# lmb-freiburg/neural-point-cloud-diffusion

Measured on AMD Instinct MI355X. Metric: denoiser train steps/sec (+ rendered rays/sec under 'render'), SRN-Cars 512pt x 128d, higher is better.
Workload: dtype bf16; 1 GPU; BASELINE configs[1]: denoiser fwd/bwd + AdamW + EMA, 512 points x 128-d latents, width 1024 / 24 layers / 16 heads (seq 513), bf16 autocast; global_batch=64, per_gpu_batch=64, parallelism=dp1, rng=weights seed 1234 on every rank; timestep / noise draws seed 42 + rank

## Files before the change

### include/npcd_hip.h

```cpp
#ifndef NPCD_HIP_H
#define NPCD_HIP_H

#include <stdint.h>

#ifdef __cplusplus
extern "C" {
#endif

#define NPCD_OK 0
#define NPCD_ERR_ARG (-1)
#define NPCD_ERR_UNSUPPORTED (-2)
#define NPCD_ERR_HIP (-3)

#define NPCD_BF16 0
#define NPCD_F16 1
#define NPCD_F32 2

int npcd_abi_version(void);
const char* npcd_error_string(int code);
const char* npcd_last_hip_error(void);

int npcd_attn_fwd(const void* q, const void* k, const void* v, void* out, float* lse,
                  int B, int n, int H, int d,
                  int64_t qkv_sb, int64_t qkv_sn, int64_t qkv_sh,
// ... 146 lines not shown
typedef struct NpcdColsumJob {
    const float* part;
    float* out;
    int nblk, N, accumulate, reserved;
} NpcdColsumJob;
int npcd_colsum_finalize_batch(const NpcdColsumJob* jobs, int njobs, void* stream);
int npcd_gelu_fwd(const void* h, void* g, int64_t numel, void* stream);
int npcd_colsum_blocks(int T);
int npcd_gelu_bwd(const void* dg, const void* h, void* dh, float* part, int T, int N, void* stream);
int npcd_colsum_bf16(const void* a, float* part, int T, int N, void* stream);
int npcd_small_wgrad_blocks(int T);
int npcd_small_wgrad(const void* dy, const void* x, float* part, int T, int J, int K, void* stream);
int npcd_adamw_ema(float* p, float* g, float* m, float* v, float* ema, void* shadow_bf16, int64_t numel,
                   float lr, float beta1, float beta2, float eps, float weight_decay, int step,
                   float ema_decay, int zero_grad, void* stream);
int npcd_cast_f32_bf16(const float* src, void* dst, int64_t numel, void* stream);
int npcd_add_ln_fwd_dt(const float* x_in, const void* delta, const float* gamma, const float* beta,
                       float* x_out, void* y, float* mean, float* rstd, int T, int W, float eps, int dtype, void* stream);
int npcd_ln_bwd_dt(const void* dy, const float* x, const float* mean, const float* rstd, const float* gamma,
                   const float* dres, float* dx, void* dxb, float* part_gamma, float* part_beta,
                   float* part_col, int T, int W, int dtype, void* stream);
int npcd_gelu_fwd_dt(const void* h, void* g, int64_t numel, int dtype, void* stream);
int npcd_gelu_bwd_dt(const void* dg, const void* h, void* dh, float* part, int T, int N, int dtype, void* stream);
int npcd_colsum_dt(const void* a, float* part, int T, int N, int dtype, void* stream);
int npcd_adamw_ema_dt(float* p, float* g, float* m, float* v, float* ema, void* shadow, int shadow_dtype, int64_t numel,
                      float lr, float beta1, float beta2, float eps, float weight_decay, int step,
                      float ema_decay, int zero_grad, void* stream);
int npcd_cast_f32_dt(const float* src, void* dst, int64_t numel, int dtype, void* stream);

typedef struct NpcdScalerCtl {
    int32_t found_inf, step, growth_tracker, skipped;
    float loss_scale, inv_scale, grad_norm, clip_coef, bc1, bc2_sqrt;
    int32_t reserved[6];
} NpcdScalerCtl;
int npcd_grad_stats_blocks(void);
int npcd_grad_stats(const float* g, int64_t n, double* work, double* out, void* stream);
int npcd_scaler_finalize(const double* stats, int nslots, NpcdScalerCtl* ctl, int scaling, int clip, float max_norm,
                         float beta1, float beta2, float growth_factor, float backoff_factor, int growth_interval, void* stream);
int npcd_adamw_ema_gated(float* p, float* g, float* m, float* v, float* ema, void* shadow, int shadow_dtype, int64_t numel,
                         float lr, float beta1, float beta2, float eps, float weight_decay, double ema_decay, int zero_grad,
                         const NpcdScalerCtl* ctl, void* stream);

int npcd_wgrad_slices(int T, int N, int K);
int npcd_wgrad(const void* dy, const void* x, float* out, float* workspace, int T, int N, int K, int dtype, void* stream);
int npcd_wgrad_group(int count, const void* const* dy, const void* const* x, float* const* out, const int* N, const int* K, int T,
                     int dtype, void* stream);

int npcd_linear_fwd(const void* x, const void* w, const void* bias, void* y, int M, int N, int K, int dtype, void* stream);
int npcd_linear_gelu_fwd(const void* x, const void* w, const void* bias, void* h, void* g, int M, int N, int K, int dtype, void* stream);
int npcd_linear_dgelu_rows(int M);
int npcd_linear_dgelu_bwd(const void* dy, const void* wt, const void* h, void* dh, float* part, int M, int N, int K, int dtype, void* stream);
int npcd_linear128_fwd(const void* x, const void* w, const void* bias, void* y, int M, int N, int K, int dtype, void* stream);
int npcd_transpose_16(const void* in, void* out, int R, int C, void* stream);

int npcd_sum_slices(const float* part, float* out, int S, int64_t numel, void* stream);

int npcd_ddpm_reverse_step(const float* x_t, const void* eps, int eps_dtype, const float* noise, float* x_prev, float* x0_out,
                           const int64_t* t, int B, int64_t per_sample, const float* tab_recip, const float* tab_recipm1,
                           const float* tab_coef1, const float* tab_coef2, const float* tab_logvar, float clip_lo, float clip_hi,
                           int has_clip, void* stream);

int npcd_q_sample(const float* x0, const float* noise, const int64_t* t, const float* tab_sqrt_acp, const float* tab_sqrt_1macp,
                  float* x_t, int B, int64_t per_sample, void* stream);
int npcd_eps_mse_blocks(void);
int npcd_eps_mse_fwd(const float* noise, const void* eps, int eps_dtype, int64_t numel, float* pointwise, float* part, float* loss,
                     void* stream);
int npcd_eps_mse_bwd(const float* noise, const void* eps, int eps_dtype, int64_t numel, const float* upstream_dev, void* grad,
                     void* stream);

int npcd_ray_march_compact(const float* sigma, const float* rgb, const uint64_t* ray_bits, const float* pts,
                           const int32_t* ray_base, const float* rays_o, const float* rays_d, const float* t1,
                           int Nr, int M, int capacity, int white_back, float* mask, float* depth, float* channels,
                           float* depth_ws, void* stream);

int64_t npcd_render_lim_words(int B, int R);
int npcd_render_rays_query(const npcd_grid_params* grid, const void* workspace, const float* points, int B, int N, const float* extr,
                           const float* intr, int views, int res, float box, int S, int M, int k, float r, float* rays_o, float* rays_d,
                           float* t0, float* t1, int32_t* counter, int32_t capacity, int32_t* ray_base, int32_t* ray_nsel,
                           uint64_t* ray_bits, int32_t* nb_idx, float* pts, void* order_ws, uint32_t* lim_part, void* stream);
int npcd_ray_march_compact_fused(const float* sigma, const float* rgb, const uint64_t* ray_bits, const float* pts, const int32_t* ray_base,
                                 const float* rays_o, const float* rays_d, const float* t0, const float* t1, const uint32_t* lim_part,
                                 int lim_pairs, int Nr, int M, int capacity, int white_back, float* mask, float* depth,
                                 float* channels, float* depth_ws, void* stream);

int npcd_pair_input_fwd(const int64_t* flat, const int64_t* owner, const float* pts, const float* kp_pos, const float* kp_feat,
                        int feat_dim, int n_freqs, int64_t n_pairs, float* x0, float* w, void* stream);
int npcd_pair_input_bwd(const int64_t* flat, const float* dx0, int feat_dim, int n_cols, int64_t n_pairs, float* dfeat, void* stream);
int npcd_leaky_bwd_blocks(int64_t rows);
int npcd_leaky_bwd_colsum(const void* dz, const void* z, void* dy, float* part, int64_t rows, int N, float slope, int dtype,
                          void* stream);
int npcd_pair_aggregate(int backward, const float* src, const float* w, const int64_t* off, const int64_t* cnt, int channels,
                        int64_t n_points, float* dst, void* stream);

#define NPCD_PAIR_MLP_BF16 0
#define NPCD_PAIR_MLP_X2 1
int64_t npcd_pair_mlp_wpack_bytes(int feat_dim, int precision);
int npcd_pair_mlp_pack(const float* const* weights_dev, const float* const* biases_dev, int feat_dim, int precision, void* wpack_dev,
                       void* stream);
int npcd_pair_mlp_fwd(const void* wpack, int feat_dim, int precision, const int64_t* nb_idx, const float* pts, const float* kp_pos,
                      const float* kp_feat, const int64_t* off, int64_t n_points, int k, int64_t n_pairs, void* x0, void* acts,
                      float* wn, float* G, void* stream);
int npcd_pair_mlp_bwd_slabs(int64_t n_pairs, int precision);
int64_t npcd_pair_mlp_bwd_workspace_floats(int feat_dim, int64_t n_pairs, int precision);
int npcd_pair_mlp_bwd(const void* wpack, int feat_dim, int precision, const float* dG, const int64_t* owner, const float* wn,
                      const void* x0, const void* acts, int64_t n_pairs, void* dact, float* dfeat, float* part, float* const* dW,
                      float* const* db, void* stream);
// ... 26 lines not shown
```

### neural-point-cloud-diffusion_amd/csrc/gemm_nt.hip

```cpp
#include <type_traits>

#include "common.h"

namespace npcd {

__device__ __forceinline__ uint32_t l_lds_addr(const unsigned char* p) {
    return (uint32_t)(uintptr_t)(__attribute__((address_space(3))) const unsigned char*)p;
}
__device__ __forceinline__ const void* l_uniform_ptr(const void* p) {
    const uint64_t v = reinterpret_cast<uint64_t>(p);
    const uint32_t lo = __builtin_amdgcn_readfirstlane((uint32_t)v), hi = __builtin_amdgcn_readfirstlane((uint32_t)(v >> 32));
    return reinterpret_cast<const void*>(((uint64_t)hi << 32) | lo);
}
__device__ __forceinline__ void l_dma16(const void* sbase, uint32_t voff, uint32_t lds_dst) {
    sbase = l_uniform_ptr(sbase);
    asm volatile("s_mov_b32 m0, %2\n\ts_nop 0\n\tglobal_load_lds_dwordx4 %0, %1" ::"v"(voff), "s"(sbase), "s"(lds_dst) : "memory");
}
__device__ __forceinline__ void l_dma16_lane(const void* src, uint32_t lds_dst) {
    asm volatile("s_mov_b32 m0, %1\n\ts_nop 0\n\tglobal_load_lds_dwordx4 %0, off" ::"v"(src), "s"(lds_dst) : "memory");
}
template <int OFF>
__device__ __forceinline__ u32x4 l_rd128(uint32_t addr) {
    u32x4 v;
    asm volatile("ds_read_b128 %0, %1 offset:%2" : "=v"(v) : "v"(addr), "n"(OFF) : "memory");
// ... 539 lines not shown
#pragma unroll
    for (int ni = 0; ni < 2; ++ni) {
        const int nb = n0 + 64 * wn + 32 * ni;
        float bq[4][4];
#pragma unroll
        for (int q = 0; q < 4; ++q) {
            if (bias) lin_unpack4<TR>(*reinterpret_cast<const u32x2*>(bias + nb + 8 * q + 4 * h), bq[q]);
            else bq[q][0] = bq[q][1] = bq[q][2] = bq[q][3] = 0.f;
        }
#pragma unroll
        for (int mi = 0; mi < MB; ++mi) {
            if (mi >= mb_store) continue;
            const int m = m0 + xrow0 + 32 * mi + r;
            const bool ok = m < p.M;
            const int64_t rowoff = (int64_t)(ok ? m : 0) * p.N + nb + 8 * h;
#pragma unroll
            for (int qp = 0; qp < 2; ++qp) {
                float v[2][4];
#pragma unroll
                for (int e = 0; e < 2; ++e)
#pragma unroll
                    for (int j = 0; j < 4; ++j) v[e][j] = acc[ni][mi][4 * (2 * qp + e) + j] + bq[2 * qp + e][j];
                const uint32_t a0 = lin_pack2<E>(v[0][0], v[0][1]), a1 = lin_pack2<E>(v[0][2], v[0][3]);
                const uint32_t b0 = lin_pack2<E>(v[1][0], v[1][1]), b1 = lin_pack2<E>(v[1][2], v[1][3]);
                const auto s0 = __builtin_amdgcn_permlane32_swap(a0, b0, false, false);
                const auto s1 = __builtin_amdgcn_permlane32_swap(a1, b1, false, false);
                if (ok) *reinterpret_cast<u32x4*>(Y + rowoff + 16 * qp) = u32x4{s0[0], s1[0], s0[1], s1[1]};
            }
        }
    }
}

template <class TR>
__global__ __launch_bounds__(512, 2) void lin128_kernel(Lin128Params p) {
    extern __shared__ __attribute__((aligned(16))) unsigned char smem[];
    const int l = xcd_remap(blockIdx.x, gridDim.x);
    const int tn = l % p.tiles_n, tm = l / p.tiles_n;
    if (p.tall && tm == p.tiles_m - 1) lin128_tile<TR, 3>(p, smem, tm, tn);
    else lin128_tile<TR, 2>(p, smem, tm, tn);
}

template <class E>
__global__ __launch_bounds__(256) void transpose16_kernel(const E* __restrict__ in, E* __restrict__ out, int R, int C) {
    __shared__ E tile[64][66];
    const int c0 = blockIdx.x * 64, r0 = blockIdx.y * 64;
    const int tx = threadIdx.x & 63, ty = threadIdx.x >> 6;
    for (int i = ty; i < 64; i += 4)
        if (r0 + i < R && c0 + tx < C) tile[i][tx] = in[(int64_t)(r0 + i) * C + c0 + tx];
    __syncthreads();
    for (int i = ty; i < 64; i += 4)
        if (c0 + i < C && r0 + tx < R) out[(int64_t)(c0 + i) * R + r0 + tx] = tile[tx][i];
}

}

using namespace npcd;

static int lin_cus() {
    static const int n = [] {
        int dev = 0, cu = 256;
        if (hipGetDevice(&dev) == hipSuccess && hipDeviceGetAttribute(&cu, hipDeviceAttributeMultiprocessorCount, dev) != hipSuccess) cu = 256;
        const char* e = getenv("NPCD_LIN_GRID");
        return e ? atoi(e) : cu;
    }();
    return n;
}

template <class TR, int EPI>
static int lin_launch(const LinParams& p, hipStream_t st) {
    static DynLds lds;
    const void* k = reinterpret_cast<const void*>(lin_kernel<TR, EPI>);
    NPCD_HIP_CHECK(lds.ensure(k, kLRing));
    const int grid = p.ntiles < lin_cus() ? p.ntiles : lin_cus();
    hipLaunchKernelGGL((lin_kernel<TR, EPI>), dim3(grid), dim3(512), kLRing, st, p);
    NPCD_HIP_CHECK(hipGetLastError());
    return NPCD_OK;
}

static int lin_common(int epi, const void* x, const void* w, const void* bias, void* y, void* y2, const void* aux, float* part, int M, int N, int K,
                      int dtype, void* stream) {
    if (!x || !w || !y || M <= 0 || N <= 0 || K <= 0) return NPCD_ERR_ARG;
    if (N % 256 || (N / 256) % 4 || K % 64 || (dtype != NPCD_BF16 && dtype != NPCD_F16)) return NPCD_ERR_UNSUPPORTED;
    if ((int64_t)M * N >= (int64_t)1 << 31 || (int64_t)M * K >= (int64_t)1 << 31) return NPCD_ERR_UNSUPPORTED;
    for (const void* q : {x, w, bias, (const void*)y, (const void*)y2, aux})
        if (reinterpret_cast<uintptr_t>(q) & 15) return NPCD_ERR_ARG;
    if (epi == LIN_GELU && !y2) return NPCD_ERR_ARG;
    if (epi == LIN_DGELU && (!aux || !part || bias)) return NPCD_ERR_ARG;
    LinParams p{};
    p.x = x; p.w = w; p.bias = bias; p.y = y; p.y2 = y2; p.aux = aux; p.part = part;
    p.M = M; p.N = N; p.K = K;
    p.tiles_m = (M + 255) / 256; p.tiles_n = N / 256;
    p.ntiles = p.tiles_m * p.tiles_n;
    p.full_m = p.tiles_m / 8 * 8;
    hipStream_t st = static_cast<hipStream_t>(stream);
#define NPCD_LIN_GO(TRT)                                                          \
    switch (epi) {                                                                \
        case LIN_PLAIN: return lin_launch<TRT, LIN_PLAIN>(p, st);                 \
        case LIN_GELU: return lin_launch<TRT, LIN_GELU>(p, st);                   \
        default: return lin_launch<TRT, LIN_DGELU>(p, st);                        \
    }
    if (dtype == NPCD_BF16) { NPCD_LIN_GO(BF16) }
    NPCD_LIN_GO(F16)
#undef NPCD_LIN_GO
}

extern "C" int npcd_linear_fwd(const void* x, const void* w, const void* bias, void* y, int M, int N, int K, int dtype, void* stream) {
    return lin_common(LIN_PLAIN, x, w, bias, y, nullptr, nullptr, nullptr, M, N, K, dtype, stream);
}
extern "C" int npcd_linear_gelu_fwd(const void* x, const void* w, const void* bias, void* h, void* g, int M, int N, int K, int dtype, void* stream) {
    return lin_common(LIN_GELU, x, w, bias, h, g, nullptr, nullptr, M, N, K, dtype, stream);
}
extern "C" int npcd_linear_dgelu_rows(int M) { return M <= 0 ? -1 : 2 * ((M + 255) / 256); }
extern "C" int npcd_linear_dgelu_bwd(const void* dy, const void* wt, const void* h, void* dh, float* part, int M, int N, int K, int dtype,
                                     void* stream) {
    return lin_common(LIN_DGELU, dy, wt, nullptr, dh, nullptr, h, part, M, N, K, dtype, stream);
}
extern "C" int npcd_linear128_fwd(const void* x, const void* w, const void* bias, void* y, int M, int N, int K, int dtype, void* stream) {
    if (!x || !w || !y || M <= 0 || N <= 0 || K <= 0) return NPCD_ERR_ARG;
    if (N % 128 || K % 64 || (dtype != NPCD_BF16 && dtype != NPCD_F16)) return NPCD_ERR_UNSUPPORTED;
    if ((int64_t)M * N >= (int64_t)1 << 31 || (int64_t)M * K >= (int64_t)1 << 30 || (int64_t)N * K >= (int64_t)1 << 30) return NPCD_ERR_UNSUPPORTED;
    for (const void* q : {x, w, bias, (const void*)y})
        if (reinterpret_cast<uintptr_t>(q) & 15) return NPCD_ERR_ARG;
    Lin128Params p{};
    p.x = x; p.w = w; p.bias = bias; p.y = y;
    p.M = M; p.N = N; p.K = K;
    const int rem = M % 128;
    p.tall = (M > 128 && rem >= 1 && rem <= 32) ? 128 + rem : 0;
    p.tiles_m = p.tall ? M / 128 : (M + 127) / 128;
    p.tiles_n = N / 128;
    hipStream_t st = static_cast<hipStream_t>(stream);
    static DynLds lds_b, lds_h;
    const int grid = p.tiles_m * p.tiles_n;
    if (dtype == NPCD_BF16) {
        NPCD_HIP_CHECK(lds_b.ensure(reinterpret_cast<const void*>(lin128_kernel<BF16>), kL128Lds));
        hipLaunchKernelGGL(lin128_kernel<BF16>, dim3(grid), dim3(512), kL128Lds, st, p);
    } else {
        NPCD_HIP_CHECK(lds_h.ensure(reinterpret_cast<const void*>(lin128_kernel<F16>), kL128Lds));
        hipLaunchKernelGGL(lin128_kernel<F16>, dim3(grid), dim3(512), kL128Lds, st, p);
    }
    NPCD_HIP_CHECK(hipGetLastError());
    return NPCD_OK;
}
#ifdef NPCD_L128_TL
extern "C" int npcd_lin128_debug_read(long long* out, int count) {
    return (int)hipMemcpyFromSymbol(out, HIP_SYMBOL(npcd::g_l128_tl), sizeof(long long) * count);
}
#endif
#ifdef NPCD_LIN_TL
extern "C" int npcd_lin_debug_read(long long* out, int count) {
    return (int)hipMemcpyFromSymbol(out, HIP_SYMBOL(npcd::g_lin_tl), sizeof(long long) * count);
}
#endif
extern "C" int npcd_transpose_16(const void* in, void* out, int R, int C, void* stream) {
    if (!in || !out || R <= 0 || C <= 0) return NPCD_ERR_ARG;
    hipLaunchKernelGGL(transpose16_kernel<uint16_t>, dim3((C + 63) / 64, (R + 63) / 64), dim3(256), 0, static_cast<hipStream_t>(stream),
                       static_cast<const uint16_t*>(in), static_cast<uint16_t*>(out), R, C);
    NPCD_HIP_CHECK(hipGetLastError());
    return NPCD_OK;
}
```

### neural-point-cloud-diffusion_amd/npcd/hip/__init__.py

```python
import ctypes
import os
from ctypes import POINTER, c_char_p, c_double, c_float, c_int, c_int32, c_int64, c_void_p

import torch

_PKG_ROOT = os.path.dirname(os.path.dirname(os.path.dirname(os.path.abspath(__file__))))
LIB_PATH = os.environ.get("NPCD_HIP_LIB") or os.path.join(_PKG_ROOT, "lib", "libnpcd_hip.so")

NPCD_BF16, NPCD_F16, NPCD_F32 = 0, 1, 2
NPCD_GRID_FINE, NPCD_GRID_SCALED = 0, 1
_DTYPE_CODE = {torch.bfloat16: NPCD_BF16, torch.float16: NPCD_F16, torch.float32: NPCD_F32}


class GridParams(ctypes.Structure):
    _fields_ = [("voxel_size", c_float * 3), ("voxel_scale", c_int32 * 3), ("kernel_size", c_int32 * 3),
                ("max_points_per_voxel", c_int32), ("max_occ_voxels_per_example", c_int32),
                ("range_min", c_float * 3), ("range_max", c_float * 3), ("dims", c_int32 * 3), ("cdims", c_int32 * 3),
                ("grid_level", c_int32)]


_P = c_void_p
SIGNATURES = {
    "npcd_abi_version": (c_int, []),
    "npcd_error_string": (c_char_p, [c_int]),
# ... 30 lines not shown
    "npcd_ray_march_compact_fused": (c_int, [_P] * 10 + [c_int, c_int, c_int, c_int, c_int] + [_P] * 4 + [_P]),
    "npcd_ray_gen": (c_int, [_P, _P, c_int, c_int, c_float] + [_P] * 5 + [_P]),
    "npcd_ray_gen_subset": (c_int, [_P, _P, c_int, c_int, c_float, _P, c_int] + [_P] * 5 + [_P]),
    "npcd_shade_wpack_bytes": (c_int64, [c_int, c_int, c_int]),
    "npcd_shade_workspace_bytes": (c_int64, [c_int, c_int]),
    "npcd_shade_pack_weights": (c_int, [POINTER(_P), POINTER(_P), c_int, c_int, c_int, _P]),
    "npcd_pairs_x2_wpack_bytes": (c_int64, [c_int]),
    "npcd_pairs_x2_pack": (c_int, [POINTER(_P), POINTER(_P), c_int, _P]),
    "npcd_pairs_x2": (c_int, [_P, c_int, _P, _P, _P, _P, _P, c_int, c_int, _P, _P]),
    "npcd_points_x2_wpack_bytes": (c_int64, []),
    "npcd_points_x2_pack": (c_int, [POINTER(_P), POINTER(_P), c_int, _P]),
    "npcd_points_x2": (c_int, [_P, _P, _P, c_int, _P, _P, _P, _P, _P]),
    "npcd_points_x2_train": (c_int, [_P, _P, c_int, _P, _P, _P]),
    "npcd_points_x2_pack_dev": (c_int, [POINTER(_P), POINTER(_P), c_int, _P, _P]),
    "npcd_shade_points": (c_int, [_P, c_int, c_int, c_int] + [_P] * 5 + [c_int, c_int] + [_P] * 3 + [_P] + [_P]),
    "npcd_shade_points_dir": (c_int, [_P, c_int, c_int, c_int] + [_P] * 5 + [c_int, c_int] + [_P] * 3 + [_P, _P] + [_P] + [_P]),
    "npcd_ray_march_ws_floats": (c_int64, [c_int]),
    "npcd_ray_gen_ws_floats": (c_int64, [c_int, c_int, c_int]),
    "npcd_ray_march": (c_int, [_P] * 8 + [c_int, c_int, c_int] + [_P] * 4 + [_P]),
    "npcd_add_ln_fwd": (c_int, [_P] * 8 + [c_int, c_int, c_float, _P]),
    "npcd_ln_bwd_blocks": (c_int, [c_int]),
    "npcd_ln_bwd": (c_int, [_P] * 11 + [c_int, c_int, _P]),
    "npcd_colsum_scratch_rows": (c_int, []),
    "npcd_colsum_finalize": (c_int, [_P, c_int, c_int, _P, c_int, _P]),
    "npcd_colsum_finalize_batch": (c_int, [_P, c_int, _P]),
    "npcd_ddpm_reverse_step": (c_int, [_P, _P, c_int, _P, _P, _P, _P, c_int, c_int64, _P, _P, _P, _P, _P, c_float, c_float, c_int, _P]),
    "npcd_gelu_fwd": (c_int, [_P, _P, c_int64, _P]),
    "npcd_colsum_blocks": (c_int, [c_int]),
    "npcd_gelu_bwd": (c_int, [_P, _P, _P, _P, c_int, c_int, _P]),
    "npcd_colsum_bf16": (c_int, [_P, _P, c_int, c_int, _P]),
    "npcd_adamw_ema": (c_int, [_P] * 6 + [c_int64] + [c_float] * 5 + [c_int, c_float, c_int, _P]),
    "npcd_cast_f32_bf16": (c_int, [_P, _P, c_int64, _P]),
    "npcd_add_ln_fwd_dt": (c_int, [_P] * 8 + [c_int, c_int, c_float, c_int, _P]),
    "npcd_ln_bwd_dt": (c_int, [_P] * 11 + [c_int, c_int, c_int, _P]),
    "npcd_gelu_fwd_dt": (c_int, [_P, _P, c_int64, c_int, _P]),
    "npcd_gelu_bwd_dt": (c_int, [_P, _P, _P, _P, c_int, c_int, c_int, _P]),
    "npcd_colsum_dt": (c_int, [_P, _P, c_int, c_int, c_int, _P]),
    "npcd_adamw_ema_dt": (c_int, [_P] * 6 + [c_int, c_int64] + [c_float] * 5 + [c_int, c_float, c_int, _P]),
    "npcd_cast_f32_dt": (c_int, [_P, _P, c_int64, c_int, _P]),
    "npcd_grad_stats_blocks": (c_int, []),
    "npcd_grad_stats": (c_int, [_P, c_int64, _P, _P, _P]),
    "npcd_scaler_finalize": (c_int, [_P, c_int, _P, c_int, c_int] + [c_float] * 5 + [c_int, _P]),
    "npcd_adamw_ema_gated": (c_int, [_P] * 6 + [c_int, c_int64] + [c_float] * 5 + [c_double, c_int, _P, _P]),
    "npcd_wgrad_slices": (c_int, [c_int, c_int, c_int]),
    "npcd_wgrad": (c_int, [_P, _P, _P, _P, c_int, c_int, c_int, c_int, _P]),
    "npcd_wgrad_group": (c_int, [c_int, POINTER(_P), POINTER(_P), POINTER(_P), POINTER(c_int), POINTER(c_int), c_int, c_int, _P]),
    "npcd_sum_slices": (c_int, [_P, _P, c_int, c_int64, _P]),
    "npcd_linear_fwd": (c_int, [_P, _P, _P, _P, c_int, c_int, c_int, c_int, _P]),
    "npcd_linear128_fwd": (c_int, [_P, _P, _P, _P, c_int, c_int, c_int, c_int, _P]),
    "npcd_linear_gelu_fwd": (c_int, [_P, _P, _P, _P, _P, c_int, c_int, c_int, c_int, _P]),
    "npcd_linear_dgelu_rows": (c_int, [c_int]),
    "npcd_linear_dgelu_bwd": (c_int, [_P, _P, _P, _P, _P, c_int, c_int, c_int, c_int, _P]),
    "npcd_transpose_16": (c_int, [_P, _P, c_int, c_int, _P]),
    "npcd_small_wgrad_blocks": (c_int, [c_int]),
    "npcd_small_wgrad": (c_int, [_P, _P, _P, c_int, c_int, c_int, _P]),
    "npcd_q_sample": (c_int, [_P] * 6 + [c_int, c_int64, _P]),
    "npcd_eps_mse_blocks": (c_int, []),
    "npcd_eps_mse_fwd": (c_int, [_P, _P, c_int, c_int64, _P, _P, _P, _P]),
    "npcd_eps_mse_bwd": (c_int, [_P, _P, c_int, c_int64, _P, _P, _P]),
    "npcd_split3_bf16": (c_int, [_P, _P, _P, c_int64, c_int, c_int, _P]),
    "npcd_add_ln_split3_bf16": (c_int, [_P] * 7 + [c_int64, c_int, c_float, _P]),
    "npcd_add_ln_split3_stats_bf16": (c_int, [_P] * 9 + [c_int64, c_int, c_float, _P]),
    "npcd_split_weights_bf16": (c_int, [_P, c_int, _P]),
    "npcd_ln_bwd_split3_bf16": (c_int, [_P] * 11 + [c_int, c_int, _P]),
    "npcd_split3_colsum_bf16": (c_int, [_P] * 5 + [c_int, c_int, c_int, _P]),
    "npcd_pair_mlp_wpack_bytes": (c_int64, [c_int, c_int]),
    "npcd_pair_mlp_pack": (c_int, [POINTER(_P), POINTER(_P), c_int, c_int, _P, _P]),
    "npcd_pair_mlp_fwd": (c_int, [_P, c_int, c_int] + [_P] * 5 + [c_int64, c_int, c_int64] + [_P] * 4 + [_P]),
    "npcd_pair_mlp_bwd_slabs": (c_int, [c_int64, c_int]),
    "npcd_pair_mlp_bwd_workspace_floats": (c_int64, [c_int, c_int64, c_int]),
    "npcd_pair_mlp_bwd": (c_int, [_P, c_int, c_int] + [_P] * 5 + [c_int64] + [_P] * 3 + [POINTER(_P), POINTER(_P), _P]),
}

_lib = None


def lib() -> ctypes.CDLL:
    global _lib
    if _lib is None:
        if not os.path.exists(LIB_PATH):
            raise RuntimeError(
                f"libnpcd_hip.so not found at {LIB_PATH}: build it with "
                f"`python neural-point-cloud-diffusion_amd/csrc/build.py` (or __graft_entry__.build()). "
                f"There is no CPU / PyTorch fallback for the NPCD hot path.")
        handle = ctypes.CDLL(LIB_PATH)
        missing = []
        for name, (res, args) in SIGNATURES.items():
            try:
                fn = getattr(handle, name)
            except AttributeError:
                missing.append(name)
                continue
            fn.restype, fn.argtypes = res, args
        handle.npcd_missing = tuple(missing)
        _lib = handle
    return _lib


def check(rc: int, what: str):
    if rc != 0:
        L = lib()
        msg = L.npcd_error_string(rc).decode()
        if rc == -3:
            msg += ": " + L.npcd_last_hip_error().decode()
        raise RuntimeError(f"{what} failed: {msg} (code {rc})")

# ... 27 lines not shown
```

### neural-point-cloud-diffusion_amd/npcd/hip/linear.py

```python
import torch

from . import arena, check, dtype_code, lib, ptr, require_gpu, stream_ptr

_f32 = torch.float32

KERNEL_EVENTS = None


def _timed(tag, fn):
    if KERNEL_EVENTS is None or tag not in KERNEL_EVENTS:
        return fn()
    e0, e1 = torch.cuda.Event(enable_timing=True), torch.cuda.Event(enable_timing=True)
    e0.record()
    rc = fn()
    e1.record()
    KERNEL_EVENTS[tag].append((e0, e1))
    return rc


def supported(M: int, N: int, K: int) -> bool:
    return M >= 1 and N % 1024 == 0 and K % 64 == 0 and M * N < 2 ** 31 and M * K < 2 ** 31


def _check_operands(x, w):
# ... 6 lines not shown

def linear_fwd(x, w, bias=None, out=None):
    _check_operands(x, w)
    M, K = x.shape
    N = w.shape[0]
    y = arena.empty((M, N), x.dtype, x.device) if out is None else out
    check(_timed("fwd", lambda: lib().npcd_linear_fwd(ptr(x), ptr(w), ptr(bias), ptr(y), M, N, K, dtype_code(x), stream_ptr())), "npcd_linear_fwd")
    return y


def supported128(M: int, N: int, K: int) -> bool:
    return M >= 1 and N % 128 == 0 and K % 64 == 0 and M * N < 2 ** 31 and M * K < 2 ** 30 and N * K < 2 ** 30


def linear128_fwd(x, w, bias=None, out=None):
    _check_operands(x, w)
    M, K = x.shape
    N = w.shape[0]
    y = arena.empty((M, N), x.dtype, x.device) if out is None else out
    check(_timed("fwd128", lambda: lib().npcd_linear128_fwd(ptr(x), ptr(w), ptr(bias), ptr(y), M, N, K, dtype_code(x), stream_ptr())), "npcd_linear128_fwd")
    return y


def linear_gelu_fwd(x, w, bias):
    _check_operands(x, w)
    M, K = x.shape
    N = w.shape[0]
    h = arena.empty((M, N), x.dtype, x.device)
    g = arena.empty_like(h)
    check(_timed("gelu_fwd", lambda: lib().npcd_linear_gelu_fwd(ptr(x), ptr(w), ptr(bias), ptr(h), ptr(g), M, N, K, dtype_code(x), stream_ptr())),
          "npcd_linear_gelu_fwd")
    return h, g


def linear_dgelu_bwd(dy, wt, h, out=None, extra_part_rows=0):
    _check_operands(dy, wt)
    M, K = dy.shape
    N = wt.shape[0]
    L = lib()
    rows = L.npcd_linear_dgelu_rows(M)
    dh = arena.empty((M, N), dy.dtype, dy.device) if out is None else out
    part = arena.empty((rows + extra_part_rows + L.npcd_colsum_scratch_rows(), N), _f32, dy.device)
    check(_timed("dgelu_bwd", lambda: L.npcd_linear_dgelu_bwd(ptr(dy), ptr(wt), ptr(h), ptr(dh), ptr(part), M, N, K, dtype_code(dy), stream_ptr())),
          "npcd_linear_dgelu_bwd")
    return dh, part, rows


def transpose16(w, out=None):
    require_gpu(w)
    R, C = w.shape
    o = arena.empty((C, R), w.dtype, w.device) if out is None else out
    check(lib().npcd_transpose_16(ptr(w), ptr(o), R, C, stream_ptr()), "npcd_transpose_16")
    return o
```

### neural-point-cloud-diffusion_amd/npcd/models/diffusion/fused.py

```python
import math

import torch

from ...hip import arena as harena
from ...hip import attention as hattn
from ...hip import elementwise as ew
from ...hip import linear as hlin

_bf16, _f32 = torch.bfloat16, torch.float32
_BLOCK_PARAMS = ("ln_1.weight", "ln_1.bias", "attn.c_qkv.weight", "attn.c_qkv.bias", "attn.c_proj.weight", "attn.c_proj.bias",
                 "ln_2.weight", "ln_2.bias", "mlp.c_fc.weight", "mlp.c_fc.bias", "mlp.c_proj.weight", "mlp.c_proj.bias")


import os


def _env_on(name):
    return os.environ.get(name, "") not in ("", "0")


_SPLIT = 0 if os.environ.get("NPCD_NO_GEMM_SPLIT") else 256
_SPLIT_MIN = int(os.environ.get("NPCD_GEMM_SPLIT_MIN", "16000"))
_SPLIT_BIG_FIRST = not os.environ.get("NPCD_GEMM_SPLIT_SMALL_FIRST")
_ATTN_COLSUM = not os.environ.get("NPCD_NO_ATTN_COLSUM")
_SUM_KERNEL = not os.environ.get("NPCD_NO_SUM_KERNEL")
_OWN_WGRAD = _env_on("NPCD_OWN_WGRAD")
_OWN_DGELU = _env_on("NPCD_OWN_DGELU")


_SPLIT_WIDE_N = int(os.environ.get("NPCD_GEMM_SPLIT_WIDE_N", "4096"))


def _split_gemm(fn, T, N=0):
    wide = _SPLIT_WIDE_N > 0 and N >= _SPLIT_WIDE_N and T > _SPLIT
    Tm = T - T % _SPLIT if (_SPLIT and (T >= _SPLIT_MIN or wide)) else T
    if Tm == 0 or Tm == T:
        fn(slice(0, T))
        return
    if _SPLIT_BIG_FIRST:
        fn(slice(0, Tm))
        fn(slice(Tm, T))
        return
    fn(slice(Tm, T))
    fn(slice(0, Tm))


_LIN128 = not os.environ.get("NPCD_NO_LIN128")
_LIN128_MAX_T = int(os.environ.get("NPCD_LIN128_MAX_T", "4200"))


def _linear(bias, x, w16):
    T = x.shape[0]
    out = harena.empty((T, w16.shape[0]), x.dtype, x.device)
    N, K = w16.shape
    if (_LIN128 and N == 1024 and K == 1024 and T <= _LIN128_MAX_T and x.is_cuda and x.is_contiguous() and w16.is_contiguous()
            and bias.is_contiguous() and x.dtype == w16.dtype == bias.dtype and hlin.supported128(T, N, K)):
        return hlin.linear128_fwd(x, w16, bias, out)
    wt = w16.t()
    _split_gemm(lambda r: torch.addmm(bias, x[r], wt, out=out[r]), T, N)
    return out


def _dgrad(dy, w16):
    T = dy.shape[0]
    out = harena.empty((T, w16.shape[1]), dy.dtype, dy.device)
    _split_gemm(lambda r: torch.mm(dy[r], w16, out=out[r]), T, w16.shape[1])
    return out


def _wgrad(dy, x, out):
    if _OWN_WGRAD and ew.wgrad(dy, x, out):
        return
    T = dy.shape[0]
    small = out.numel() <= (1 << 20)
    S = 8 if small else 4
    S = min(S, max(1, T // (2048 if small else 4096)))
    while S > 1 and T % S:
        S //= 2
    if S == 1:
        torch.mm(dy.t(), x, out_dtype=_f32, out=out)
        return
    part = torch.bmm(dy.view(S, T // S, -1).transpose(1, 2), x.view(S, T // S, -1), out_dtype=_f32)
    if not (_SUM_KERNEL and ew.sum_slices(part, out)):
        torch.sum(part, dim=0, out=out)


def _parse_wgrad_stream(value):
    if value is None or value == "":
        return True, 20000
    if value == "0":
        return False, 0
    if value == "1":
        return True, 1 << 62
    try:
        return True, int(value)
    except ValueError:
        raise ValueError(f"NPCD_WGRAD_STREAM={value!r}: expected unset, 0 (off), 1 (on at every size) or a token-row limit") from None


_WGRAD_STREAM, _WGRAD_STREAM_MAX_T = _parse_wgrad_stream(os.environ.get("NPCD_WGRAD_STREAM"))
_side = {}


def _side_stream(device):
    s = _side.get(device)
    if s is None:
        s = _side[device] = torch.cuda.Stream(device=device, priority=int(os.environ.get("NPCD_WGRAD_STREAM_PRIO", "0")))
    return s


def _wgrad_side_ok(T):
    return _WGRAD_STREAM and T <= _WGRAD_STREAM_MAX_T


_WGRAD_GROUP = os.environ.get("NPCD_WGRAD_GROUP", "1") != "0"
_WGRAD_GROUP_MAX_T = int(os.environ.get("NPCD_WGRAD_GROUP_MAX_T", "17000"))
_JOIN_PER_BLOCK = _env_on("NPCD_WGRAD_JOIN_PER_BLOCK")
_STEP_ARENA = os.environ.get("NPCD_STEP_ARENA", "1") != "0"
_STEP_ARENA_MAX_T = int(os.environ.get("NPCD_STEP_ARENA_MAX_T", "20000"))
# ... 25 lines not shown

import contextlib

_NULL = contextlib.nullcontext()


class _BlockViews:
    fp32_class = False

    def __deepcopy__(self, memo):
        return None

    def __reduce__(self):
        return (_no_engine, ())

    def __init__(self, backbone, flat, reducer=None):
        self.heads = backbone.resblocks[0].attn.heads
        self.width = backbone.width
        self.reducer = reducer
        self._offset = {id(p): off for p, off in zip(flat.params, flat.offsets)}
        self.blocks = []
        for blk in backbone.resblocks:
            named = dict(blk.named_parameters())
            entry = {"params": [named[n] for n in _BLOCK_PARAMS]}
            for n in _BLOCK_PARAMS:
                p = named[n]
                off = self._offset[id(p)]
                key = n.replace(".", "_")
                entry[key] = p.data
                entry[key + "_g"] = flat.grad[off:off + p.numel()].view_as(p)
            self.blocks.append(entry)
        self.block_ranges, self.wait_range = None, None

    def shadow_written(self):
        pass


class FusedBackboneEngine(_BlockViews):

    def __init__(self, backbone, flat, shadow, reducer=None):
        super().__init__(backbone, flat, reducer)
        for blk, entry in zip(backbone.resblocks, self.blocks):
            named = dict(blk.named_parameters())
            for n in _BLOCK_PARAMS:
                p = named[n]
                off = self._offset[id(p)]
                entry[n.replace(".", "_") + "_16"] = shadow[off:off + p.numel()].view_as(p)

        self._flat, self._shadow = flat, shadow
        self.dtype = shadow.dtype
        self._stamped = [p for e in self.blocks for p in e["params"]]
        self._stamp = self._versions()
        self.shadow_epoch = 0
        self.arena = harena.StepArena() if _STEP_ARENA else None

    def shadow_written(self):
        self.shadow_epoch += 1

    def _versions(self):
        return [p._version for p in self._stamped]

    def sync_shadow(self, force=False):
        v = self._versions()
        if force or v != self._stamp:
            if self.wait_range is not None:
                self.wait_range()
            for p, off in zip(self._flat.params, self._flat.offsets):
                if p.data_ptr() != self._flat.flat.data_ptr() + off * self._flat.flat.element_size():
                    raise RuntimeError("a parameter of the fused backbone was re-homed outside the trainer's flat buffer "
                                       "(p.data replaced): build a new DiffusionTrainer for this model")
            ew.cast_f32_bf16(self._flat.flat, self._shadow)
            self.shadow_written()
            self._stamp = v

    def __call__(self, x):
        self.sync_shadow()
        return _BackboneFn.apply(x, self)


class InferenceWeights:

    def __init__(self, backbone):
        self.heads = backbone.resblocks[0].attn.heads
        self.params = [[dict(blk.named_parameters())[n] for n in _BLOCK_PARAMS] for blk in backbone.resblocks]
        self.stamp, self.blocks = None, None

    def current(self):
        stamp = [(p._version, p.data_ptr()) for ps in self.params for p in ps]
        if stamp != self.stamp:
            self.blocks = []
            for ps in self.params:
                e = {}
                for n, p in zip(_BLOCK_PARAMS, ps):
                    key = n.replace(".", "_")
                    e[key] = p.data
                    if not n.startswith("ln_"):
                        e[key + "_16"] = p.data.to(_bf16)
                self.blocks.append(e)
            self.stamp = stamp
        return self.blocks


class InferenceWeightsX2:

    def __init__(self, backbone):
        self.heads = backbone.resblocks[0].attn.heads
        self.params = [[dict(blk.named_parameters())[n] for n in _BLOCK_PARAMS] for blk in backbone.resblocks]
        self.stamp, self.blocks = None, None

    def current(self):
# ... 46 lines not shown
    return xs.view(B, n, W)


def backbone_forward(x, blocks, heads, dtype=_bf16):
    B, n, W = x.shape
    T, d = B * n, W // heads
    scale = 1.0 / math.sqrt(d)
    with torch.autocast("cuda", enabled=False):
        xs = x.reshape(T, W).contiguous()
        delta = None
        for e in blocks:
            x1, y1, _, _ = ew.add_ln_fwd(xs, delta, e["ln_1_weight"], e["ln_1_bias"], dtype=dtype)
            x_cur = xs if x1 is None else x1
            q4 = _linear(e["attn_c_qkv_bias_16"], y1, e["attn_c_qkv_weight_16"]).view(B, n, heads, 3 * d)
            a, _ = hattn._fwd(q4[..., :d], q4[..., d:2 * d], q4[..., 2 * d:], scale)
            o = _linear(e["attn_c_proj_bias_16"], a.view(T, W), e["attn_c_proj_weight_16"])
            xs, y2, _, _ = ew.add_ln_fwd(x_cur, o, e["ln_2_weight"], e["ln_2_bias"])
            g = ew.gelu_fwd(_linear(e["mlp_c_fc_bias_16"], y2, e["mlp_c_fc_weight_16"]))
            delta = _linear(e["mlp_c_proj_bias_16"], g, e["mlp_c_proj_weight_16"])
        out = xs + delta
    return out.view(B, n, W)


class _BackboneFn(torch.autograd.Function):
    @staticmethod
    def forward(ctx, x, eng):
        B, n, W = x.shape
        T = B * n
        arena = eng.arena if (eng.arena is not None and x.is_cuda and T <= _STEP_ARENA_MAX_T) else None
        token = arena.begin() if arena is not None else 0
        if not token:
            arena = None
        ctx.arena, ctx.arena_token = arena, token
        if arena is None:
            return _BackboneFn._forward(ctx, x, eng)
        ctx.arena_guard = harena.StepGuard(arena, token)
        try:
            with arena.active():
                return _BackboneFn._forward(ctx, x, eng)
        except BaseException:
            arena.end(token)
            raise

    @staticmethod
    def _forward(ctx, x, eng):
        B, n, W = x.shape
        T, H = B * n, eng.heads
        d = W // H
        scale = 1.0 / math.sqrt(d)
        saved = []
        with torch.autocast("cuda", enabled=False):
            xs = x.reshape(T, W).contiguous()
            delta = None
            for bi, e in enumerate(eng.blocks):
                if eng.wait_range is not None:
                    eng.wait_range(*eng.block_ranges[bi])
                x1, y1, mean1, rstd1 = ew.add_ln_fwd(xs, delta, e["ln_1_weight"], e["ln_1_bias"], dtype=eng.dtype)
                x_cur = xs if x1 is None else x1
                qkv = _linear(e["attn_c_qkv_bias_16"], y1, e["attn_c_qkv_weight_16"])
                q4 = qkv.view(B, n, H, 3 * d)
                a, lse = hattn._fwd(q4[..., :d], q4[..., d:2 * d], q4[..., 2 * d:], scale)
                a = a.view(T, W)
                o = _linear(e["attn_c_proj_bias_16"], a, e["attn_c_proj_weight_16"])
                x2, y2, mean2, rstd2 = ew.add_ln_fwd(x_cur, o, e["ln_2_weight"], e["ln_2_bias"])
                h = _linear(e["mlp_c_fc_bias_16"], y2, e["mlp_c_fc_weight_16"])
                g = ew.gelu_fwd(h)
                delta = _linear(e["mlp_c_proj_bias_16"], g, e["mlp_c_proj_weight_16"])
                saved.append((x_cur, mean1, rstd1, y1, qkv, a, lse, x2, mean2, rstd2, y2, h, g))
                xs = x2
            out = xs + delta
        ctx.eng, ctx.saved, ctx.dims, ctx.scale = eng, saved, (B, n, W, H, d), scale
        return out.view(B, n, W)

    @staticmethod
    def backward(ctx, dout):
        if any(s is None for s in ctx.saved):
            raise RuntimeError("the fused backbone engine does not support retain_graph / double backward: run a new forward "
                               "for every backward")
        arena = ctx.arena
        if arena is None:
            return _BackboneFn._backward(ctx, dout)
        try:
            with arena.active():
                return _BackboneFn._backward(ctx, dout)
        finally:
            arena.end(ctx.arena_token)

    @staticmethod
    def _backward(ctx, dout):
        eng, (B, n, W, H, d), scale = ctx.eng, ctx.dims, ctx.scale
        T = B * n
        with torch.autocast("cuda", enabled=False):
            dx = dout.reshape(T, W).contiguous().float()
            dxb = dx.to(eng.dtype)
            last = eng.blocks[-1]
            last["mlp_c_proj_bias_g"].copy_(dx.sum(dim=0))
            side, pending = _wgrad_side_ok(T), []

            reducing = eng.reducer is not None and eng.reducer.active

            def ready(entry):
                if reducing:
                    for p in entry["params"]:
                        eng.reducer.mark_ready(p)
            for bi in range(len(eng.blocks) - 1, -1, -1):
                e = eng.blocks[bi]
                x_cur, mean1, rstd1, y1, qkv, a, lse, x2, mean2, rstd2, y2, h, g = ctx.saved[bi]
                ctx.saved[bi] = None
                sums = ew.ColsumBatch()
                wg = pending.append if side else (lambda t: _wgrad(*t))
                Tm = T - T % 256
                w2 = e["mlp_c_proj_weight_16"]
                if (_OWN_DGELU and Tm > 0 and hlin.supported(Tm, 4 * W, W) and dxb.is_contiguous() and h.is_contiguous()
                        and w2.is_contiguous() and dxb.dtype == w2.dtype == h.dtype and dxb.dtype in (torch.bfloat16, torch.float16)):
                    wT = e.get("mlp_c_proj_weight_16T")
                    if wT is None or e.get("mlp_c_proj_weight_16T_epoch") != eng.shadow_epoch or wT.dtype != w2.dtype:
                        with harena.paused():
                            wT = e["mlp_c_proj_weight_16T"] = hlin.transpose16(w2, out=wT if wT is not None and wT.dtype == w2.dtype else None)
                        e["mlp_c_proj_weight_16T_epoch"] = eng.shadow_epoch
                    dh = harena.empty_like(h)
                    extra = ew.lib().npcd_colsum_blocks(T - Tm) if Tm < T else 0
                    _, part, rows = hlin.linear_dgelu_bwd(dxb[:Tm], wT, h[:Tm], out=dh[:Tm], extra_part_rows=extra)
                    if Tm < T:
                        dg = torch.mm(dxb[Tm:], e["mlp_c_proj_weight_16"])
                        ew.gelu_bwd(dg, h[Tm:], None, out=dh[Tm:], part_rows=part[rows:])
                        del dg
                    sums.add(part, rows + extra, 4 * W, e["mlp_c_fc_bias_g"])
                    wg((dxb, g, e["mlp_c_proj_weight_g"]))
                    del g, h
                else:
                    dg = _dgrad(dxb, e["mlp_c_proj_weight_16"])
                    wg((dxb, g, e["mlp_c_proj_weight_g"]))
                    dh = ew.gelu_bwd(dg, h, e["mlp_c_fc_bias_g"], batch=sums)
                    del dg, g, h
                dy2 = _dgrad(dh, e["mlp_c_fc_weight_16"])
                wg((dh, y2, e["mlp_c_fc_weight_g"]))
                del dh, y2
                dx2, dx2b = ew.ln_bwd(dy2, x2, mean2, rstd2, e["ln_2_weight"], dx, e["ln_2_weight_g"], e["ln_2_bias_g"],
                                      e["attn_c_proj_bias_g"], batch=sums)
                del dy2, x2, dx, dxb
                da = _dgrad(dx2b, e["attn_c_proj_weight_16"])
                wg((dx2b, a, e["attn_c_proj_weight_g"]))
                dqkv = harena.empty_like(qkv)
                q4, g4 = qkv.view(B, n, H, 3 * d), dqkv.view(B, n, H, 3 * d)
                cpart = hattn.colsum_part_for(g4[..., :d]) if _ATTN_COLSUM else None
                hattn._bwd(q4[..., :d], q4[..., d:2 * d], q4[..., 2 * d:], a.view(B, n, H, d), da.view(B, n, H, d), lse,
                           g4[..., :d], g4[..., d:2 * d], g4[..., 2 * d:], scale, colsum_part=cpart[0] if cpart else None)
                del da, a, qkv, dx2b
                if cpart:
                    sums.add(cpart[0], cpart[1], 3 * W, e["attn_c_qkv_bias_g"])
                else:
                    ew.colsum_bf16(dqkv, e["attn_c_qkv_bias_g"], batch=sums)
                dy1 = _dgrad(dqkv, e["attn_c_qkv_weight_16"])
                wg((dqkv, y1, e["attn_c_qkv_weight_g"]))
                del dqkv, y1
                prev_bias_g = eng.blocks[bi - 1]["mlp_c_proj_bias_g"] if bi > 0 else None
                with (harena.paused() if bi == 0 else _NULL):
                    dx, dxb = ew.ln_bwd(dy1, x_cur, mean1, rstd1, e["ln_1_weight"], dx2, e["ln_1_weight_g"], e["ln_1_bias_g"],
                                        prev_bias_g, want_bf16=bi > 0, batch=sums)
                del dy1, dx2
                sums.flush()
                if side and _JOIN_PER_BLOCK:
                    if bi + 1 < len(eng.blocks):
                        _wgrad_join(dx.device)
                        ready(eng.blocks[bi + 1])
                    _wgrad_fork(pending, dx.device)
                elif side:
                    above = eng.blocks[bi + 1] if (reducing and bi + 1 < len(eng.blocks)) else None
                    _wgrad_fork(pending, dx.device, before=None if above is None else (lambda: ready(above)))
                else:
                    ready(e)
            if side:
                _wgrad_join(dx.device)
                ready(eng.blocks[0])
        return dx.view(B, n, W), None


SPLIT_WIDTHS = (256, 512, 768, 1024, 2048)
_X2_LINEARS = ("attn_c_qkv", "attn_c_proj", "mlp_c_fc", "mlp_c_proj")


def x2_supported(width, heads):
    if heads <= 0 or width % heads or width // heads != 64:
        return (f"head dim {width // heads if heads > 0 and width % heads == 0 else width / max(heads, 1)}: the fp32 attention backward "
                f"is built for head dim 64 only")
    if width not in SPLIT_WIDTHS:
        return f"width {width}: the split-operand kernels take widths {', '.join(map(str, SPLIT_WIDTHS))}"
    return None


def _mm_x2(a3, w3):
    return torch.mm(a3, w3, out_dtype=_f32)


def _wgrad_x2(dy3, x3, out):
    T, N = dy3.shape[0], out.shape[0]
    K = out.shape[1]
    d, x = dy3.view(T, 3, N), x3.view(T, 3, K)
    part = harena.empty((3, N, K), _f32, out.device)
    torch.bmm(d[:, 0:2].permute(1, 2, 0), x[:, 1:3].permute(1, 0, 2), out_dtype=_f32, out=part[0:2])
    torch.mm(d[:, 0].t(), x[:, 0], out_dtype=_f32, out=part[2])
    torch.sum(part, dim=0, out=out)


_X2_WGRAD = os.environ.get("NPCD_X2_WGRAD", "library")
if _X2_WGRAD not in ("library", "own"):
# ... 124 lines not shown
```

Before: 12.19 steps/s.

## Pre-transpose block weights each forward for NT-layout dgrad GEMMs in backward

Adds a grouped 16-bit transpose kernel (vectorized, swizzled LDS tile) that transposes all four linear weights of a block in one launch during the forward pass, caching them per shadow epoch. In the backward pass, the dgrad GEMMs then multiply by wT.t() so that hipBLAS sees a different (transposed-contiguous) operand layout, which is meant to pick a faster GEMM variant for large token counts (T ≥ 16000 by default; here T=64*513≈32.8k). This replaces the ad-hoc per-block transpose of only the MLP projection weight. The cost is extra transpose work and memory per step, and a dependency on the transposed layout actually being faster for rocBLAS/hipBLASLt.

```diff
diff --git a/include/npcd_hip.h b/include/npcd_hip.h
--- a/include/npcd_hip.h
+++ b/include/npcd_hip.h
@@ -222,6 +222,7 @@
 int npcd_linear_dgelu_bwd(const void* dy, const void* wt, const void* h, void* dh, float* part, int M, int N, int K, int dtype, void* stream);
 int npcd_linear128_fwd(const void* x, const void* w, const void* bias, void* y, int M, int N, int K, int dtype, void* stream);
 int npcd_transpose_16(const void* in, void* out, int R, int C, void* stream);
+int npcd_transpose16_group(int count, const void* const* in, void* const* out, const int* R, const int* C, void* stream);
 
 int npcd_sum_slices(const float* part, float* out, int S, int64_t numel, void* stream);
 
diff --git a/neural-point-cloud-diffusion_amd/csrc/gemm_nt.hip b/neural-point-cloud-diffusion_amd/csrc/gemm_nt.hip
--- a/neural-point-cloud-diffusion_amd/csrc/gemm_nt.hip
+++ b/neural-point-cloud-diffusion_amd/csrc/gemm_nt.hip
@@ -615,6 +615,62 @@
         if (c0 + i < C && r0 + tx < R) out[(int64_t)(c0 + i) * R + r0 + tx] = tile[tx][i];
 }
 
+constexpr int kTransposeGroupMax = 4;
+struct TransposeGroup {
+    const uint16_t* in[kTransposeGroupMax];
+    uint16_t* out[kTransposeGroupMax];
+    int R[kTransposeGroupMax], C[kTransposeGroupMax];
+    int first[kTransposeGroupMax + 1];
+    int count;
+};
+
+__device__ __forceinline__ int transpose_slot(int c, int r) { return c * 64 + ((((r >> 3) ^ (c >> 3)) & 7) << 3) + (r & 7); }
+
+__global__ __launch_bounds__(256) void transpose16_group_kernel(TransposeGroup gp) {
+    __shared__ __attribute__((aligned(16))) uint16_t tile[64 * 64];
+    const int w = blockIdx.x;
+    int g = 0;
+#pragma unroll
+    for (int i = 1; i < kTransposeGroupMax; ++i)
+        if (i < gp.count && w >= gp.first[i]) g = i;
+    const uint16_t* __restrict__ in = gp.in[g];
+    uint16_t* __restrict__ out = gp.out[g];
+    const int R = gp.R[g], C = gp.C[g];
+    const int tiles_c = (C + 63) >> 6, t = w - gp.first[g];
+    const int r0 = (t / tiles_c) * 64, c0 = (t % tiles_c) * 64;
+    const bool full = r0 + 64 <= R && c0 + 64 <= C;
+    const bool wide_in = full && !(reinterpret_cast<uintptr_t>(in) & 15) && !(C & 7);
+    const bool wide_out = full && !(reinterpret_cast<uintptr_t>(out) & 15) && !(R & 7);
+    const int tid = threadIdx.x;
+    if (wide_in) {
+        const int cg = tid & 7, rp = tid >> 3;
+        const uint16_t* src = in + (int64_t)(r0 + 2 * rp) * C + c0 + 8 * cg;
+        const u32x4 a = *reinterpret_cast<const u32x4*>(src), b = *reinterpret_cast<const u32x4*>(src + C);
+        uint32_t* image = reinterpret_cast<uint32_t*>(tile);
+#pragma unroll
+        for (int j = 0; j < 8; ++j) {
+            const uint32_t lo = (j & 1) ? a[j >> 1] >> 16 : a[j >> 1] & 0xffffu;
+            const uint32_t hi = (j & 1) ? b[j >> 1] & 0xffff0000u : b[j >> 1] << 16;
+            image[transpose_slot(8 * cg + j, 2 * rp) >> 1] = lo | hi;
+        }
+    } else {
+        const int tx = tid & 63, ty = tid >> 6;
+        for (int i = ty; i < 64; i += 4)
+            if (r0 + i < R && c0 + tx < C) tile[transpose_slot(tx, i)] = in[(int64_t)(r0 + i) * C + c0 + tx];
+    }
+    __syncthreads();
+    if (wide_out) {
+        const int rg = tid & 7;
+#pragma unroll
+        for (int c = tid >> 3; c < 64; c += 32)
+            *reinterpret_cast<u32x4*>(out + (int64_t)(c0 + c) * R + r0 + 8 * rg) = *reinterpret_cast<const u32x4*>(tile + transpose_slot(c, 8 * rg));
+    } else {
+        const int tx = tid & 63, ty = tid >> 6;
+        for (int i = ty; i < 64; i += 4)
+            if (c0 + i < C && r0 + tx < R) out[(int64_t)(c0 + i) * R + r0 + tx] = tile[transpose_slot(i, tx)];
+    }
+}
+
 }
 
 using namespace npcd;
@@ -721,3 +777,21 @@
     NPCD_HIP_CHECK(hipGetLastError());
     return NPCD_OK;
 }
+extern "C" int npcd_transpose16_group(int count, const void* const* in, void* const* out, const int* R, const int* C, void* stream) {
+    if (count < 1 || count > kTransposeGroupMax || !in || !out || !R || !C) return NPCD_ERR_ARG;
+    TransposeGroup gp{};
+    gp.count = count;
+    int64_t tiles = 0;
+    for (int g = 0; g < count; ++g) {
+        if (!in[g] || !out[g] || R[g] <= 0 || C[g] <= 0) return NPCD_ERR_ARG;
+        if ((reinterpret_cast<uintptr_t>(in[g]) & 1) || (reinterpret_cast<uintptr_t>(out[g]) & 1)) return NPCD_ERR_ARG;
+        gp.in[g] = static_cast<const uint16_t*>(in[g]); gp.out[g] = static_cast<uint16_t*>(out[g]); gp.R[g] = R[g]; gp.C[g] = C[g];
+        gp.first[g] = (int)tiles;
+        tiles += (int64_t)((R[g] + 63) / 64) * ((C[g] + 63) / 64);
+        if (tiles >= (int64_t)1 << 31) return NPCD_ERR_UNSUPPORTED;
+    }
+    gp.first[count] = (int)tiles;
+    hipLaunchKernelGGL(transpose16_group_kernel, dim3((unsigned)tiles), dim3(256), 0, static_cast<hipStream_t>(stream), gp);
+    NPCD_HIP_CHECK(hipGetLastError());
+    return NPCD_OK;
+}
diff --git a/neural-point-cloud-diffusion_amd/npcd/hip/__init__.py b/neural-point-cloud-diffusion_amd/npcd/hip/__init__.py
--- a/neural-point-cloud-diffusion_amd/npcd/hip/__init__.py
+++ b/neural-point-cloud-diffusion_amd/npcd/hip/__init__.py
@@ -106,6 +106,7 @@
     "npcd_linear_dgelu_rows": (c_int, [c_int]),
     "npcd_linear_dgelu_bwd": (c_int, [_P, _P, _P, _P, _P, c_int, c_int, c_int, c_int, _P]),
     "npcd_transpose_16": (c_int, [_P, _P, c_int, c_int, _P]),
+    "npcd_transpose16_group": (c_int, [c_int, POINTER(_P), POINTER(_P), POINTER(c_int), POINTER(c_int), _P]),
     "npcd_small_wgrad_blocks": (c_int, [c_int]),
     "npcd_small_wgrad": (c_int, [_P, _P, _P, c_int, c_int, c_int, _P]),
     "npcd_q_sample": (c_int, [_P] * 6 + [c_int, c_int64, _P]),
diff --git a/neural-point-cloud-diffusion_amd/npcd/hip/linear.py b/neural-point-cloud-diffusion_amd/npcd/hip/linear.py
--- a/neural-point-cloud-diffusion_amd/npcd/hip/linear.py
+++ b/neural-point-cloud-diffusion_amd/npcd/hip/linear.py
@@ -82,3 +82,19 @@
     o = arena.empty((C, R), w.dtype, w.device) if out is None else out
     check(lib().npcd_transpose_16(ptr(w), ptr(o), R, C, stream_ptr()), "npcd_transpose_16")
     return o
+
+
+def transpose16_group(pairs):
+    import ctypes
+    n = len(pairs)
+    for w, o in pairs:
+        require_gpu(w, o)
+        if (w.dim() != 2 or w.element_size() != 2 or o.dtype != w.dtype or tuple(o.shape) != (w.shape[1], w.shape[0])
+                or not w.is_contiguous() or not o.is_contiguous()):
+            raise RuntimeError("npcd transpose16_group: contiguous 16-bit w [R, C] and out [C, R] of one type expected, got "
+                               f"{tuple(w.shape)} {w.dtype} -> {tuple(o.shape)} {o.dtype}")
+    P = ctypes.c_void_p * n
+    I = ctypes.c_int * n
+    check(lib().npcd_transpose16_group(n, P(*[ptr(w) for w, _ in pairs]), P(*[ptr(o) for _, o in pairs]),
+                                       I(*[w.shape[0] for w, _ in pairs]), I(*[w.shape[1] for w, _ in pairs]), stream_ptr()),
+          "npcd_transpose16_group")
diff --git a/neural-point-cloud-diffusion_amd/npcd/models/diffusion/fused.py b/neural-point-cloud-diffusion_amd/npcd/models/diffusion/fused.py
--- a/neural-point-cloud-diffusion_amd/npcd/models/diffusion/fused.py
+++ b/neural-point-cloud-diffusion_amd/npcd/models/diffusion/fused.py
@@ -10,6 +10,7 @@
 _bf16, _f32 = torch.bfloat16, torch.float32
 _BLOCK_PARAMS = ("ln_1.weight", "ln_1.bias", "attn.c_qkv.weight", "attn.c_qkv.bias", "attn.c_proj.weight", "attn.c_proj.bias",
                  "ln_2.weight", "ln_2.bias", "mlp.c_fc.weight", "mlp.c_fc.bias", "mlp.c_proj.weight", "mlp.c_proj.bias")
+_LINEARS = ("attn_c_qkv", "attn_c_proj", "mlp_c_fc", "mlp_c_proj")
 
 
 import os
@@ -26,6 +27,8 @@
 _SUM_KERNEL = not os.environ.get("NPCD_NO_SUM_KERNEL")
 _OWN_WGRAD = _env_on("NPCD_OWN_WGRAD")
 _OWN_DGELU = _env_on("NPCD_OWN_DGELU")
+_DGRAD_NN = _env_on("NPCD_DGRAD_NN")
+_DGRAD_T_MIN_T = int(os.environ.get("NPCD_DGRAD_T_MIN_T", "16000"))
 
 
 _SPLIT_WIDE_N = int(os.environ.get("NPCD_GEMM_SPLIT_WIDE_N", "4096"))
@@ -61,10 +64,11 @@
     return out
 
 
-def _dgrad(dy, w16):
+def _dgrad(dy, w16, wT=None):
     T = dy.shape[0]
     out = harena.empty((T, w16.shape[1]), dy.dtype, dy.device)
-    _split_gemm(lambda r: torch.mm(dy[r], w16, out=out[r]), T, w16.shape[1])
+    b = w16 if wT is None else wT.t()
+    _split_gemm(lambda r: torch.mm(dy[r], b, out=out[r]), T, w16.shape[1])
     return out
 
 
@@ -196,10 +200,37 @@
         self._stamped = [p for e in self.blocks for p in e["params"]]
         self._stamp = self._versions()
         self.shadow_epoch = 0
+        self._shadowT, self._wT = None, None
+        self._wT_stamp = [None] * len(self.blocks)
+        self.transposed_refreshes = 0
         self.arena = harena.StepArena() if _STEP_ARENA else None
 
     def shadow_written(self):
         self.shadow_epoch += 1
+
+    def wants_transposed(self, T):
+        return _OWN_DGELU or (not _DGRAD_NN and T >= _DGRAD_T_MIN_T)
+
+    def refresh_transposed(self, bi):
+        if self._wT_stamp[bi] == self.shadow_epoch:
+            return
+        if self._shadowT is None:
+            sizes = [entry[k + "_weight_16"].numel() for entry in self.blocks for k in _LINEARS]
+            self._shadowT = torch.empty(sum(sizes), dtype=self._shadow.dtype, device=self._shadow.device)
+            self._wT, off = [], 0
+            for entry in self.blocks:
+                views = []
+                for k in _LINEARS:
+                    N, K = entry[k + "_weight_16"].shape
+                    views.append(self._shadowT[off:off + N * K].view(K, N))
+                    off += N * K
+                self._wT.append(views)
+        e = self.blocks[bi]
+        hlin.transpose16_group([(e[k + "_weight_16"], v) for k, v in zip(_LINEARS, self._wT[bi])])
+        for k, v in zip(_LINEARS, self._wT[bi]):
+            e[k + "_weight_16T"] = v
+        self._wT_stamp[bi] = self.shadow_epoch
+        self.transposed_refreshes += 1
 
     def _versions(self):
         return [p._version for p in self._stamped]
@@ -352,9 +383,12 @@
         with torch.autocast("cuda", enabled=False):
             xs = x.reshape(T, W).contiguous()
             delta = None
+            ctx.transposed = transposed = x.is_cuda and eng.wants_transposed(T)
             for bi, e in enumerate(eng.blocks):
                 if eng.wait_range is not None:
                     eng.wait_range(*eng.block_ranges[bi])
+                if transposed:
+                    eng.refresh_transposed(bi)
                 x1, y1, mean1, rstd1 = ew.add_ln_fwd(xs, delta, e["ln_1_weight"], e["ln_1_bias"], dtype=eng.dtype)
                 x_cur = xs if x1 is None else x1
                 qkv = _linear(e["attn_c_qkv_bias_16"], y1, e["attn_c_qkv_weight_16"])
@@ -396,6 +430,7 @@
             last = eng.blocks[-1]
             last["mlp_c_proj_bias_g"].copy_(dx.sum(dim=0))
             side, pending = _wgrad_side_ok(T), []
+            dgrad_t = ctx.transposed and not _DGRAD_NN and T >= _DGRAD_T_MIN_T
 
             reducing = eng.reducer is not None and eng.reducer.active
 
@@ -411,35 +446,31 @@
                 wg = pending.append if side else (lambda t: _wgrad(*t))
                 Tm = T - T % 256
                 w2 = e["mlp_c_proj_weight_16"]
-                if (_OWN_DGELU and Tm > 0 and hlin.supported(Tm, 4 * W, W) and dxb.is_contiguous() and h.is_contiguous()
+                if (_OWN_DGELU and ctx.transposed and Tm > 0 and hlin.supported(Tm, 4 * W, W) and dxb.is_contiguous() and h.is_contiguous()
                         and w2.is_contiguous() and dxb.dtype == w2.dtype == h.dtype and dxb.dtype in (torch.bfloat16, torch.float16)):
-                    wT = e.get("mlp_c_proj_weight_16T")
-                    if wT is None or e.get("mlp_c_proj_weight_16T_epoch") != eng.shadow_epoch or wT.dtype != w2.dtype:
-                        with harena.paused():
-                            wT = e["mlp_c_proj_weight_16T"] = hlin.transpose16(w2, out=wT if wT is not None and wT.dtype == w2.dtype else None)
-                        e["mlp_c_proj_weight_16T_epoch"] = eng.shadow_epoch
+                    wT = e["mlp_c_proj_weight_16T"]
                     dh = harena.empty_like(h)
                     extra = ew.lib().npcd_colsum_blocks(T - Tm) if Tm < T else 0
                     _, part, rows = hlin.linear_dgelu_bwd(dxb[:Tm], wT, h[:Tm], out=dh[:Tm], extra_part_rows=extra)
                     if Tm < T:
-                        dg = torch.mm(dxb[Tm:], e["mlp_c_proj_weight_16"])
+                        dg = torch.mm(dxb[Tm:], wT.t() if dgrad_t else w2)
                         ew.gelu_bwd(dg, h[Tm:], None, out=dh[Tm:], part_rows=part[rows:])
                         del dg
                     sums.add(part, rows + extra, 4 * W, e["mlp_c_fc_bias_g"])
                     wg((dxb, g, e["mlp_c_proj_weight_g"]))
                     del g, h
                 else:
-                    dg = _dgrad(dxb, e["mlp_c_proj_weight_16"])
+                    dg = _dgrad(dxb, w2, e["mlp_c_proj_weight_16T"] if dgrad_t else None)
                     wg((dxb, g, e["mlp_c_proj_weight_g"]))
                     dh = ew.gelu_bwd(dg, h, e["mlp_c_fc_bias_g"], batch=sums)
                     del dg, g, h
-                dy2 = _dgrad(dh, e["mlp_c_fc_weight_16"])
+                dy2 = _dgrad(dh, e["mlp_c_fc_weight_16"], e["mlp_c_fc_weight_16T"] if dgrad_t else None)
                 wg((dh, y2, e["mlp_c_fc_weight_g"]))
                 del dh, y2
                 dx2, dx2b = ew.ln_bwd(dy2, x2, mean2, rstd2, e["ln_2_weight"], dx, e["ln_2_weight_g"], e["ln_2_bias_g"],
                                       e["attn_c_proj_bias_g"], batch=sums)
                 del dy2, x2, dx, dxb
-                da = _dgrad(dx2b, e["attn_c_proj_weight_16"])
+                da = _dgrad(dx2b, e["attn_c_proj_weight_16"], e["attn_c_proj_weight_16T"] if dgrad_t else None)
                 wg((dx2b, a, e["attn_c_proj_weight_g"]))
                 dqkv = harena.empty_like(qkv)
                 q4, g4 = qkv.view(B, n, H, 3 * d), dqkv.view(B, n, H, 3 * d)
@@ -451,7 +482,7 @@
                     sums.add(cpart[0], cpart[1], 3 * W, e["attn_c_qkv_bias_g"])
                 else:
                     ew.colsum_bf16(dqkv, e["attn_c_qkv_bias_g"], batch=sums)
-                dy1 = _dgrad(dqkv, e["attn_c_qkv_weight_16"])
+                dy1 = _dgrad(dqkv, e["attn_c_qkv_weight_16"], e["attn_c_qkv_weight_16T"] if dgrad_t else None)
                 wg((dqkv, y1, e["attn_c_qkv_weight_g"]))
                 del dqkv, y1
                 prev_bias_g = eng.blocks[bi - 1]["mlp_c_proj_bias_g"] if bi > 0 else None
```

Result: faster. 12.43 steps/s, median of 6 (+1.9%).
